# callmeray/PointMVSNet

Measured on AMD Instinct MI355X. Metric: depth-maps/sec (DTU 640x512, 3 src views, 2 flow iters), higher is better.
Workload: dtype f32

## Files before the change

pointmvsnet_amd/csrc/conv3d.hip:

```cpp
#include <stdlib.h>

#include "pf_common.h"
#include "pf_bn_resolve.h"

namespace {

typedef float f32x4 __attribute__((ext_vector_type(4)));

struct ConvGeom {
  int Cin, Cout, Di, Hi, Wi, Do, Ho, Wo;
  int ID, IH, IW, IWP, plane;
  int tiles_d, tiles_h, tiles_w;
  int aff_mode, sps, aff_off;
  const float* in_scale;
  const float* in_shift;
  pf_bn_job in_bn;
};

template <int STRIDE, int TD>
struct Stage {
  static constexpr int ID = (TD - 1) * STRIDE + 3;
  static constexpr int IH = 3 * STRIDE + 3;
  static constexpr int IW = 15 * STRIDE + 3;
  static constexpr int IWP = IW + 1;
  static constexpr int RAW = ID * IH * IWP;
  static constexpr int WANT = STRIDE == 1 ? 16 : 17;
  static constexpr int PLANE = RAW + ((WANT - RAW % 32) + 32) % 32;
  static constexpr int ELEMS = ID * IH * IW;
  static constexpr int NXR = (ELEMS + 63) / 64;
};

template <int NT, int STRIDE, int TD, int MINW>
__global__ __launch_bounds__(256, MINW) void conv3d_k3_kernel(const float* __restrict__ x, const float* __restrict__ wp,
                                                        float* __restrict__ y, ConvGeom g,
                                                        double* __restrict__ partials) {
  using St = Stage<STRIDE, TD>;
  constexpr int ID = St::ID, IH = St::IH, IW = St::IW, IWP = St::IWP, PLANE = St::PLANE;
  constexpr int ELEMS = St::ELEMS, NXR = St::NXR;
  constexpr int NCP = NT * 16;
  constexpr int WSZ = 27 * 4 * NCP;
  constexpr int NWR = (WSZ + 255) / 256;
  constexpr int XS = 4 * PLANE;
  extern __shared__ __attribute__((aligned(16))) float lds[];
  float* xs0 = lds;
  float* ws0 = lds + 2 * XS;
  float* tile = lds;
  double* red = reinterpret_cast<double*>(tile + 4 * NCP * 17 + ((4 * NCP * 17) & 1));

  const int tid = threadIdx.x;
  const int wave = __builtin_amdgcn_readfirstlane(tid >> 6), lane = tid & 63;
  const int li = lane & 15, lk = lane >> 4;
  unsigned xb_, xn_;
  pf_xcd_xy<PF_XCD_CONV3D>(xb_, xn_);
  const int n = (int)xn_, bx = (int)xb_;
  const int plane_i = g.Hi * g.Wi, vol_i = plane_i * g.Di;
  const int64_t plane_o = (int64_t)g.Ho * g.Wo, vol_o = plane_o * g.Do;
  const float* xb = x + (int64_t)n * g.Cin * vol_i;
  float* yb = y + (int64_t)n * g.Cout * vol_o;
  const int cgroups = g.Cin >> 2;

  double ssum[NT], ssq[NT];
#pragma unroll
  for (int t = 0; t < NT; ++t) ssum[t] = ssq[t] = 0.0;

  float* aff = lds + g.aff_off;
  if (g.aff_mode == 1) {
    const int stat = n / g.sps;
    for (int e = tid; e < 2 * g.Cin; e += 256)
      aff[e] = e < g.Cin ? g.in_scale[(int64_t)stat * g.Cin + e] : g.in_shift[(int64_t)stat * g.Cin + e - g.Cin];
  } else if (g.aff_mode == 2) {
    pf_bn_resolve<256>(g.in_bn, n / g.sps, aff, aff + g.Cin, reinterpret_cast<double*>(lds));
  }

  const int total = g.tiles_d * g.tiles_h * g.tiles_w;
  for (int item = bx; item < total; item += gridDim.x) {
    const int tw = item % g.tiles_w;
    const int rest = item / g.tiles_w;
    const int th = rest % g.tiles_h;
    const int td = rest / g.tiles_h;
    const int od0 = td * TD, oh0 = th * 4, ow0 = tw * 16;
    const int id0 = od0 * STRIDE - 1, ih0 = oh0 * STRIDE - 1, iw0 = ow0 * STRIDE - 1;

    unsigned gofs[NXR];
    unsigned okmask = 0;
#pragma unroll
    for (int r = 0; r < NXR; ++r) {
      const int e = lane + 64 * r;
      const int row = e / IW, col = e - row * IW;
      const int dz = row / IH, hy = row - dz * IH;
      const int id = id0 + dz, ih = ih0 + hy, iw = iw0 + col;
      const bool ok = e < ELEMS && id >= 0 && id < g.Di && ih >= 0 && ih < g.Hi && iw >= 0 && iw < g.Wi;
      gofs[r] = ok ? (unsigned)(id * plane_i + ih * g.Wi + iw) : 0u;
      okmask |= (ok ? 1u : 0u) << r;
    }

    float rx[NXR], rw[NWR];
    auto load_group = [&](int cg) {
      const float* src = xb + (int64_t)(cg * 4 + wave) * vol_i;
#pragma unroll
      for (int r = 0; r < NXR; ++r) rx[r] = src[gofs[r]];
      const float* wsrc = wp + (int64_t)cg * WSZ;
#pragma unroll
      for (int r = 0; r < NWR; ++r) {
        const int e = tid + 256 * r;
        rw[r] = (256 * (r + 1) <= WSZ || e < WSZ) ? wsrc[e] : 0.0f;
      }
    };
    auto store_group = [&](int buf, int cg) {
      float* xs = xs0 + buf * XS + wave * PLANE;
      float* ws = ws0 + buf * WSZ;
      float sa = 1.0f, sb = 0.0f;
      if (g.aff_mode) {
        sa = aff[cg * 4 + wave];
        sb = aff[g.Cin + cg * 4 + wave];
      }
#pragma unroll
      for (int r = 0; r < NXR; ++r) {
        const int e = lane + 64 * r;
        float v = rx[r];
        if (g.aff_mode) v = fmaxf(fmaf(v, sa, sb), 0.0f);
        if (64 * (r + 1) <= ELEMS || e < ELEMS) xs[e + e / IW] = ((okmask >> r) & 1u) ? v : 0.0f;
      }
#pragma unroll
      for (int r = 0; r < NWR; ++r) {
        const int e = tid + 256 * r;
        if (256 * (r + 1) <= WSZ || e < WSZ) ws[e] = rw[r];
      }
    };

    f32x4 acc[TD][NT];
#pragma unroll
    for (int d = 0; d < TD; ++d)
#pragma unroll
      for (int t = 0; t < NT; ++t) acc[d][t] = (f32x4){0.0f, 0.0f, 0.0f, 0.0f};

    __syncthreads();
    load_group(0);
    store_group(0, 0);
    __syncthreads();
    for (int cg = 0; cg < cgroups; ++cg) {
      const int buf = cg & 1;
      if (cg + 1 < cgroups) load_group(cg + 1);
      const float* xs = xs0 + buf * XS + lk * PLANE + (wave * STRIDE) * IWP + li * STRIDE;
      const float* ws = ws0 + buf * WSZ + lk * NCP + li;
#pragma unroll
      for (int kd = 0; kd < 3; ++kd) {
#pragma unroll
        for (int kh = 0; kh < 3; ++kh) {
#pragma unroll
          for (int kw = 0; kw < 3; ++kw) {
            const int tap = (kd * 3 + kh) * 3 + kw;
            float b[NT];
#pragma unroll
            for (int t = 0; t < NT; ++t) b[t] = ws[tap * 4 * NCP + 16 * t];
#pragma unroll
            for (int d = 0; d < TD; ++d) {
              const float a = xs[((d * STRIDE + kd) * IH + kh) * IWP + kw];
#pragma unroll
              for (int t = 0; t < NT; ++t) acc[d][t] = __builtin_amdgcn_mfma_f32_16x16x4f32(a, b[t], acc[d][t], 0, 0, 0);
            }
          }
        }
      }
      if (cg + 1 < cgroups) store_group(buf ^ 1, cg + 1);
      __syncthreads();
    }

    const int oh = oh0 + wave;
    float* tl = tile + wave * NCP * 17;
#pragma unroll
    for (int d = 0; d < TD; ++d) {
      const int od = od0 + d;
      const bool row_ok = oh < g.Ho && od < g.Do;
#pragma unroll
      for (int t = 0; t < NT; ++t) {
        float s = 0.0f, q = 0.0f;
#pragma unroll
        for (int r = 0; r < 4; ++r) {
          const int pos = lk * 4 + r;
          const float v = acc[d][t][r];
          tl[(16 * t + li) * 17 + pos] = v;
          if (row_ok && ow0 + pos < g.Wo) {
            s += v;
            q += v * v;
          }
        }
        s += __shfl_xor(s, 16);
        q += __shfl_xor(q, 16);
        s += __shfl_xor(s, 32);
        q += __shfl_xor(q, 32);
        ssum[t] += (double)s;
        ssq[t] += (double)q;
      }
      __builtin_amdgcn_wave_barrier();
      if (row_ok) {
        for (int e = lane; e < NCP * 16; e += 64) {
          const int co = e >> 4, pos = e & 15;
          if (co < g.Cout && ow0 + pos < g.Wo)
            yb[(int64_t)co * vol_o + (int64_t)od * plane_o + (int64_t)oh * g.Wo + ow0 + pos] = tl[co * 17 + pos];
        }
      }
      __builtin_amdgcn_wave_barrier();
    }
  }

  if (partials != nullptr) {
#pragma unroll
    for (int t = 0; t < NT; ++t) {
      if (lane < 16) {
        red[((wave * NCP) + 16 * t + lane) * 2 + 0] = ssum[t];
        red[((wave * NCP) + 16 * t + lane) * 2 + 1] = ssq[t];
      }
    }
    __syncthreads();
    if (tid < g.Cout) {
      double s = 0.0, q = 0.0;
#pragma unroll
      for (int w = 0; w < 4; ++w) {
        s += red[((w * NCP) + tid) * 2 + 0];
        q += red[((w * NCP) + tid) * 2 + 1];
      }
      double* o = partials + (((int64_t)n * gridDim.x + bx) * g.Cout + tid) * 2;
      o[0] = s;
      o[1] = q;
    }
  }
}

template <int COUT>
__global__ __launch_bounds__(256) void conv3d_k3_few_kernel(const float* __restrict__ x, const float* __restrict__ w,
                                                            float* __restrict__ y, int Cin, int D, int H, int W) {
  extern __shared__ __attribute__((aligned(16))) float wl[];
  for (int e = threadIdx.x; e < COUT * Cin * 27; e += 256) wl[e] = w[e];
  __syncthreads();
  const int64_t plane = (int64_t)H * W, vol = plane * D;
  const int64_t i = (int64_t)blockIdx.x * 256 + threadIdx.x;
  const int n = blockIdx.y;
  if (i >= vol) return;
  const int od = (int)(i / plane);
  const int rem = (int)(i - (int64_t)od * plane);
  const int oh = rem / W, ow = rem - oh * W;
  float acc[COUT];
#pragma unroll
  for (int c = 0; c < COUT; ++c) acc[c] = 0.0f;
  const float* xb = x + (int64_t)n * Cin * vol;
  for (int ci = 0; ci < Cin; ++ci) {
    const float* xc = xb + (int64_t)ci * vol;
#pragma unroll
    for (int kd = 0; kd < 3; ++kd) {
      const int id = od + kd - 1;
      const bool dok = id >= 0 && id < D;
#pragma unroll
      for (int kh = 0; kh < 3; ++kh) {
        const int ih = oh + kh - 1;
        const bool hok = dok && ih >= 0 && ih < H;
        const float* row = xc + (int64_t)id * plane + (int64_t)ih * W;
#pragma unroll
        for (int kw = 0; kw < 3; ++kw) {
          const int iw = ow + kw - 1;
          const float v = (hok && iw >= 0 && iw < W) ? row[iw] : 0.0f;
#pragma unroll
          for (int c = 0; c < COUT; ++c) acc[c] = fmaf(v, wl[(c * Cin + ci) * 27 + (kd * 3 + kh) * 3 + kw], acc[c]);
        }
      }
    }
  }
#pragma unroll
  for (int c = 0; c < COUT; ++c) y[((int64_t)n * COUT + c) * vol + i] = acc[c];
}

ConvGeom make_geom(int64_t Cin, int64_t Cout, int64_t Di, int64_t Hi, int64_t Wi, int stride, int td) {
  ConvGeom g;
  g.Cin = (int)Cin;
  g.Cout = (int)Cout;
  g.Di = (int)Di;
  g.Hi = (int)Hi;
  g.Wi = (int)Wi;
  g.Do = (int)((Di - 1) / stride + 1);
  g.Ho = (int)((Hi - 1) / stride + 1);
  g.Wo = (int)((Wi - 1) / stride + 1);
  g.ID = (td - 1) * stride + 3;
  g.IH = 3 * stride + 3;
  g.IW = 15 * stride + 3;
  g.IWP = g.IW + 1;
  const int raw = g.ID * g.IH * g.IWP;
  const int want = stride == 1 ? 16 : 17;
  g.plane = raw + ((want - raw % 32) + 32) % 32;
  g.tiles_d = (g.Do + td - 1) / td;
  g.tiles_h = (g.Ho + 3) / 4;
  g.tiles_w = (g.Wo + 15) / 16;
  g.aff_mode = 0;
  g.sps = 1;
  g.aff_off = 0;
  g.in_scale = g.in_shift = nullptr;
  g.in_bn = pf_bn_job{};
  return g;
}

constexpr size_t kMaxLds = 80 * 1024;

size_t lds_work_bytes(const ConvGeom& g, int NT) {
  const int NCP = NT * 16;
  const size_t staging = sizeof(float) * (size_t)(2 * 4 * g.plane + 2 * 27 * 4 * NCP);
  const size_t epilogue = sizeof(float) * (size_t)(4 * NCP * 17 + 1) + sizeof(double) * (size_t)(4 * NCP * 2);
  const size_t m = staging > epilogue ? staging : epilogue;
  return (m + 15) / 16 * 16;
}
size_t lds_bytes_for(const ConvGeom& g, int NT) {
  return lds_work_bytes(g, NT) + sizeof(float) * 2 * (size_t)g.Cin;
}

int pick_td(int64_t Cin, int64_t Cout, int64_t Di, int64_t Hi, int64_t Wi, int stride) {
  const int NT = (int)((Cout + 15) / 16);
  int best = 0;
  for (int td = (stride == 1 && NT > 1) ? 4 : 2; td >= 1; td >>= 1) {
    const ConvGeom g = make_geom(Cin, Cout, Di, Hi, Wi, stride, td);
    if (lds_bytes_for(g, NT) > kMaxLds) continue;
    best = td;
    if ((int64_t)g.tiles_d * g.tiles_h * g.tiles_w >= 512) return td;
  }
  return best;
}

int blocks_for(const ConvGeom& g) {
  const int64_t total = (int64_t)g.tiles_d * g.tiles_h * g.tiles_w;
#ifndef PF_CONV3D_CAP
#define PF_CONV3D_CAP 2048
#endif
  if (total <= PF_CONV3D_CAP) return (int)total;
  const int64_t per = (total + PF_CONV3D_CAP - 1) / PF_CONV3D_CAP;
  return (int)((total + per - 1) / per);
}

template <int NT, int STRIDE, int TD, int MINW>
int launch(const float* x, const float* wp, float* y, const ConvGeom& g, int64_t N, double* partials,
           hipStream_t s) {
  const size_t lds_bytes = lds_bytes_for(g, NT);
  if (lds_bytes > kMaxLds) return PF_ERR_UNSUPPORTED;
  ConvGeom gk = g;
  gk.aff_off = (int)(lds_work_bytes(g, NT) / sizeof(float));
  if (lds_bytes > 64 * 1024) {
    static std::atomic<unsigned long long> done{0};
    const int rc = pf_allow_big_lds(reinterpret_cast<const void*>(&conv3d_k3_kernel<NT, STRIDE, TD, MINW>),
                                    (int)kMaxLds, done);
    if (rc != PF_OK) return rc;
  }
  dim3 grid((unsigned)blocks_for(g), (unsigned)N);
  hipLaunchKernelGGL((conv3d_k3_kernel<NT, STRIDE, TD, MINW>), grid, dim3(256), lds_bytes, s, x, wp, y, gk, partials);
  return pf_launch_status();
}

template <int NT, int STRIDE, int TD>
int launch_w(const float* x, const float* wp, float* y, const ConvGeom& g, int64_t N, double* partials,
             hipStream_t s) {
  constexpr int kDefault = (NT == 1 && STRIDE == 1 && TD == 2) ? 4 : 2;
  return launch<NT, STRIDE, TD, kDefault>(x, wp, y, g, N, partials, s);
}

template <int NT, int STRIDE>
int launch_td(int td, const float* x, const float* wp, float* y, const ConvGeom& g, int64_t N, double* partials,
              hipStream_t s) {
  if constexpr (STRIDE == 1) {
    if (td == 4) return launch_w<NT, STRIDE, 4>(x, wp, y, g, N, partials, s);
  }
  if (td == 2) return launch_w<NT, STRIDE, 2>(x, wp, y, g, N, partials, s);
  return launch_w<NT, STRIDE, 1>(x, wp, y, g, N, partials, s);
}

}

extern "C" {

int pf_conv3d_blocks(int64_t Cin, int64_t Cout, int64_t Di, int64_t Hi, int64_t Wi, int stride) {
  if (Cin <= 0 || Cout <= 0 || Di <= 0 || Hi <= 0 || Wi <= 0 || (stride != 1 && stride != 2)) return 0;
  const int td = pick_td(Cin, Cout, Di, Hi, Wi, stride);
  if (td == 0) return 0;
  return blocks_for(make_geom(Cin, Cout, Di, Hi, Wi, stride, td));
}

int pf_conv3d_k3_f32(const float* x, const float* wp, float* y, int64_t N, int64_t Cin, int64_t Cout, int64_t Di,
                     int64_t Hi, int64_t Wi, int stride, const float* in_scale, const float* in_shift,
                     const pf_bn_job* in_bn, int samples_per_stat, double* partials, void* stream) {
  PF_REQUIRE(N >= 0 && Cin >= 4 && Cout >= 1 && Di >= 1 && Hi >= 1 && Wi >= 1 && N <= 65535);
  PF_REQUIRE(stride == 1 || stride == 2);
  PF_REQUIRE(samples_per_stat >= 1 && (in_scale == nullptr) == (in_shift == nullptr));
  PF_REQUIRE(in_bn == nullptr || in_scale == nullptr);
  if (in_bn != nullptr && N > 0) {
    PF_REQUIRE(N % samples_per_stat == 0);
    const int rc = pf_bn_in_check(in_bn, (int)Cin, (int)(N / samples_per_stat));
    if (rc != PF_OK) return rc;
  }
  if ((Cin % 4) != 0 || Cout > 32) return PF_ERR_UNSUPPORTED;
  PF_REQUIRE(Cin * Di * Hi * Wi <= INT32_MAX);
  if (N == 0) return PF_OK;
  PF_REQUIRE(x && wp && y);
  const int td = pick_td(Cin, Cout, Di, Hi, Wi, stride);
  if (td == 0) return PF_ERR_UNSUPPORTED;
  ConvGeom g = make_geom(Cin, Cout, Di, Hi, Wi, stride, td);
  g.aff_mode = in_bn ? 2 : (in_scale ? 1 : 0);
  g.sps = samples_per_stat;
  g.in_scale = in_scale;
  g.in_shift = in_shift;
  if (in_bn) g.in_bn = *in_bn;
  hipStream_t s = (hipStream_t)stream;
  const int NT = (int)((Cout + 15) / 16);
  if (stride == 1)
    return NT == 1 ? launch_td<1, 1>(td, x, wp, y, g, N, partials, s) : launch_td<2, 1>(td, x, wp, y, g, N, partials, s);
  return NT == 1 ? launch_td<1, 2>(td, x, wp, y, g, N, partials, s) : launch_td<2, 2>(td, x, wp, y, g, N, partials, s);
}

int pf_conv3d_k3_few_f32(const float* x, const float* w, float* y, int64_t N, int64_t Cin, int64_t Cout, int64_t D,
                         int64_t H, int64_t W, void* stream) {
  PF_REQUIRE(N >= 0 && Cin >= 1 && Cout >= 1 && D >= 1 && H >= 1 && W >= 1 && N <= 65535);
  if (Cout > 4 || Cout * Cin * 27 * sizeof(float) > 48 * 1024) return PF_ERR_UNSUPPORTED;
  PF_REQUIRE(H * W <= INT32_MAX);
  if (N == 0) return PF_OK;
  PF_REQUIRE(x && w && y);
  const size_t lds = sizeof(float) * (size_t)(Cout * Cin * 27);
  dim3 grid((unsigned)pf_cdiv(D * H * W, 256), (unsigned)N);
  hipStream_t s = (hipStream_t)stream;
  switch ((int)Cout) {
    case 1: hipLaunchKernelGGL(conv3d_k3_few_kernel<1>, grid, dim3(256), lds, s, x, w, y, (int)Cin, (int)D, (int)H, (int)W); break;
    case 2: hipLaunchKernelGGL(conv3d_k3_few_kernel<2>, grid, dim3(256), lds, s, x, w, y, (int)Cin, (int)D, (int)H, (int)W); break;
    case 3: hipLaunchKernelGGL(conv3d_k3_few_kernel<3>, grid, dim3(256), lds, s, x, w, y, (int)Cin, (int)D, (int)H, (int)W); break;
    default: hipLaunchKernelGGL(conv3d_k3_few_kernel<4>, grid, dim3(256), lds, s, x, w, y, (int)Cin, (int)D, (int)H, (int)W); break;
  }
  return pf_launch_status();
}

}
```

pointmvsnet_amd/csrc/conv3d_pair.hip:

```cpp
#include <stdlib.h>

#include "pf_common.h"

namespace {

typedef float f32x4 __attribute__((ext_vector_type(4)));

struct PairGeom {
  int Cin, Cout, D, H, W;
  int tiles_d, tiles_h, tiles_w;
};

template <int TD>
struct PStage {
  static constexpr int ID = TD + 2;
  static constexpr int IH = 10;
  static constexpr int IW = 18;
  static constexpr int IWP = IW + 1;
  static constexpr int RAW = ID * IH * IWP;
  static constexpr int PLANE = RAW + ((16 - RAW % 32) + 32) % 32;
  static constexpr int ELEMS = ID * IH * IW;
  static constexpr int NXR = (ELEMS + 63) / 64;
};

constexpr int kTaps = 36;
constexpr int kWsz = kTaps * 4 * 16;

template <int TD>
constexpr size_t pair_lds_bytes() {
  using St = PStage<TD>;
  const size_t staging = sizeof(float) * (size_t)(2 * 4 * St::PLANE + 2 * kWsz);
  const size_t epilogue = sizeof(float) * (size_t)(4 * 16 * 17 + 1) + sizeof(double) * (size_t)(4 * 16 * 2);
  return staging > epilogue ? staging : epilogue;
}

template <int TD, int MINW>
__global__ __launch_bounds__(256, MINW) void conv3d_k3_pair_kernel(const float* __restrict__ x,
                                                                   const float* __restrict__ wp,
                                                                   float* __restrict__ y, PairGeom g,
                                                                   double* __restrict__ partials) {
  using St = PStage<TD>;
  constexpr int ID = St::ID, IH = St::IH, IW = St::IW, IWP = St::IWP, PLANE = St::PLANE;
  constexpr int ELEMS = St::ELEMS, NXR = St::NXR;
  constexpr int NWR = (kWsz + 255) / 256;
  constexpr int XS = 4 * PLANE;
  extern __shared__ __attribute__((aligned(16))) float lds[];
  float* xs0 = lds;
  float* ws0 = lds + 2 * XS;
  float* tile = lds;
  double* red = reinterpret_cast<double*>(tile + 4 * 16 * 17 + ((4 * 16 * 17) & 1));

  const int tid = threadIdx.x;
  const int wave = __builtin_amdgcn_readfirstlane(tid >> 6), lane = tid & 63;
  const int li = lane & 15, lk = lane >> 4;
  unsigned xb_, xn_;
  pf_xcd_xy<PF_XCD_CONV3D>(xb_, xn_);
  const int n = (int)xn_, bx = (int)xb_;
  const int plane_i = g.H * g.W, vol = plane_i * g.D;
  const float* xb = x + (int64_t)n * g.Cin * vol;
  float* yb = y + (int64_t)n * g.Cout * vol;
  const int cgroups = g.Cin >> 2;

  double ssum = 0.0, ssq = 0.0;

  const int total = g.tiles_d * g.tiles_h * g.tiles_w;
  for (int item = bx; item < total; item += gridDim.x) {
    const int tw = item % g.tiles_w;
    const int rest = item / g.tiles_w;
    const int th = rest % g.tiles_h;
    const int td = rest / g.tiles_h;
    const int od0 = td * TD, oh0 = th * 8, ow0 = tw * 16;
    const int id0 = od0 - 1, ih0 = oh0 - 1, iw0 = ow0 - 1;

    unsigned gofs[NXR];
    unsigned okmask = 0;
#pragma unroll
    for (int r = 0; r < NXR; ++r) {
      const int e = lane + 64 * r;
      const int row = e / IW, col = e - row * IW;
      const int dz = row / IH, hy = row - dz * IH;
      const int id = id0 + dz, ih = ih0 + hy, iw = iw0 + col;
      const bool ok = e < ELEMS && id >= 0 && id < g.D && ih >= 0 && ih < g.H && iw >= 0 && iw < g.W;
      gofs[r] = ok ? (unsigned)(id * plane_i + ih * g.W + iw) : 0u;
      okmask |= (ok ? 1u : 0u) << r;
    }

    float rx[NXR], rw[NWR];
    auto load_group = [&](int cg) {
      const float* src = xb + (int64_t)(cg * 4 + wave) * vol;
#pragma unroll
      for (int r = 0; r < NXR; ++r) rx[r] = src[gofs[r]];
      const float* wsrc = wp + (int64_t)cg * kWsz;
#pragma unroll
      for (int r = 0; r < NWR; ++r) {
        const int e = tid + 256 * r;
        rw[r] = (256 * (r + 1) <= kWsz || e < kWsz) ? wsrc[e] : 0.0f;
      }
    };
    auto store_group = [&](int buf) {
      float* xs = xs0 + buf * XS + wave * PLANE;
      float* ws = ws0 + buf * kWsz;
#pragma unroll
      for (int r = 0; r < NXR; ++r) {
        const int e = lane + 64 * r;
        if (64 * (r + 1) <= ELEMS || e < ELEMS) xs[e + e / IW] = ((okmask >> r) & 1u) ? rx[r] : 0.0f;
      }
#pragma unroll
      for (int r = 0; r < NWR; ++r) {
        const int e = tid + 256 * r;
        if (256 * (r + 1) <= kWsz || e < kWsz) ws[e] = rw[r];
      }
    };

    f32x4 acc[TD];
#pragma unroll
    for (int d = 0; d < TD; ++d) acc[d] = (f32x4){0.0f, 0.0f, 0.0f, 0.0f};

    __syncthreads();
    load_group(0);
    store_group(0);
    __syncthreads();
    for (int cg = 0; cg < cgroups; ++cg) {
      const int buf = cg & 1;
      if (cg + 1 < cgroups) load_group(cg + 1);
      const float* xs = xs0 + buf * XS + lk * PLANE + (2 * wave) * IWP + li;
      const float* ws = ws0 + buf * kWsz + lk * 16 + li;
#pragma unroll
      for (int kd = 0; kd < 3; ++kd) {
#pragma unroll
        for (int kh = 0; kh < 4; ++kh) {
#pragma unroll
          for (int kw = 0; kw < 3; ++kw) {
            const int tap = (kd * 4 + kh) * 3 + kw;
            const float b = ws[tap * 4 * 16];
#pragma unroll
            for (int d = 0; d < TD; ++d) {
              const float a = xs[((d + kd) * IH + kh) * IWP + kw];
              acc[d] = __builtin_amdgcn_mfma_f32_16x16x4f32(a, b, acc[d], 0, 0, 0);
            }
          }
        }
      }
      if (cg + 1 < cgroups) store_group(buf ^ 1);
      __syncthreads();
    }

    const int oh = oh0 + 2 * wave + (li >> 3);
    float* tl = tile + wave * 16 * 17;
#pragma unroll
    for (int d = 0; d < TD; ++d) {
      const int od = od0 + d;
      const bool row_ok = oh < g.H && od < g.D;
      float s = 0.0f, q = 0.0f;
#pragma unroll
      for (int r = 0; r < 4; ++r) {
        const int pos = lk * 4 + r;
        const float v = acc[d][r];
        tl[li * 17 + pos] = v;
        if (row_ok && ow0 + pos < g.W) {
          s += v;
          q += v * v;
        }
      }
      s += __shfl_xor(s, 8);
      q += __shfl_xor(q, 8);
      s += __shfl_xor(s, 16);
      q += __shfl_xor(q, 16);
      s += __shfl_xor(s, 32);
      q += __shfl_xor(q, 32);
      ssum += (double)s;
      ssq += (double)q;
      __builtin_amdgcn_wave_barrier();
      if (od < g.D) {
        for (int e = lane; e < 16 * 16; e += 64) {
          const int col = e >> 4, pos = e & 15;
          const int co = col & 7, ohh = oh0 + 2 * wave + (col >> 3);
          if (co < g.Cout && ohh < g.H && ow0 + pos < g.W)
            yb[(int64_t)co * vol + (int64_t)od * plane_i + (int64_t)ohh * g.W + ow0 + pos] = tl[col * 17 + pos];
        }
      }
      __builtin_amdgcn_wave_barrier();
    }
  }

  if (partials != nullptr) {
    if (lane < 8) {
      red[(wave * 16 + lane) * 2 + 0] = ssum;
      red[(wave * 16 + lane) * 2 + 1] = ssq;
    }
    __syncthreads();
    if (tid < g.Cout) {
      double s = 0.0, q = 0.0;
#pragma unroll
      for (int w = 0; w < 4; ++w) {
        s += red[(w * 16 + tid) * 2 + 0];
        q += red[(w * 16 + tid) * 2 + 1];
      }
      double* o = partials + (((int64_t)n * gridDim.x + bx) * g.Cout + tid) * 2;
      o[0] = s;
      o[1] = q;
    }
  }
}

#ifndef PF_PAIR_TD
#define PF_PAIR_TD 2
#endif
#ifndef PF_PAIR_MINW
#define PF_PAIR_MINW 3
#endif
constexpr int kPairTD = PF_PAIR_TD;

PairGeom make_pair_geom(int64_t Cin, int64_t Cout, int64_t D, int64_t H, int64_t W) {
  PairGeom g;
  g.Cin = (int)Cin;
  g.Cout = (int)Cout;
  g.D = (int)D;
  g.H = (int)H;
  g.W = (int)W;
  g.tiles_d = (g.D + kPairTD - 1) / kPairTD;
  g.tiles_h = (g.H + 7) / 8;
  g.tiles_w = (g.W + 15) / 16;
  return g;
}

int pair_blocks(const PairGeom& g) {
  const int64_t total = (int64_t)g.tiles_d * g.tiles_h * g.tiles_w;
#ifndef PF_CONV3D_CAP
#define PF_CONV3D_CAP 2048
#endif
  if (total <= PF_CONV3D_CAP) return (int)total;
  const int64_t per = (total + PF_CONV3D_CAP - 1) / PF_CONV3D_CAP;
  return (int)((total + per - 1) / per);
}

}

extern "C" {

int pf_conv3d_pair_blocks(int64_t Cin, int64_t Cout, int64_t D, int64_t H, int64_t W) {
  if (Cin <= 0 || Cout <= 0 || Cout > 8 || D <= 0 || H <= 0 || W <= 0) return 0;
  return pair_blocks(make_pair_geom(Cin, Cout, D, H, W));
}

int pf_conv3d_k3_pair_f32(const float* x, const float* wp, float* y, int64_t N, int64_t Cin, int64_t Cout, int64_t D,
                          int64_t H, int64_t W, double* partials, void* stream) {
  PF_REQUIRE(N >= 0 && Cin >= 4 && Cout >= 1 && D >= 1 && H >= 1 && W >= 1 && N <= 65535);
  if ((Cin % 4) != 0 || Cout > 8) return PF_ERR_UNSUPPORTED;
  PF_REQUIRE(Cin * D * H * W <= INT32_MAX);
  if (N == 0) return PF_OK;
  PF_REQUIRE(x && wp && y);
  const PairGeom g = make_pair_geom(Cin, Cout, D, H, W);
  constexpr size_t lds_bytes = pair_lds_bytes<kPairTD>();
  static_assert(lds_bytes <= 64 * 1024, "pair tile must fit the default dynamic LDS limit");
  dim3 grid((unsigned)pair_blocks(g), (unsigned)N);
  hipLaunchKernelGGL((conv3d_k3_pair_kernel<kPairTD, PF_PAIR_MINW>), grid, dim3(256), lds_bytes, (hipStream_t)stream, x, wp, y, g,
                     partials);
  return pf_launch_status();
}

}
```

pointmvsnet_amd/csrc/pf_common.h:

```cpp
#pragma once

#include <hip/hip_runtime.h>
#include <stdint.h>

#include "pointflow_hip.h"

#define PF_WAVE 64

unsigned* pf_status_ptr();

#define PF_REQUIRE(cond)                 \
  do {                                   \
    if (!(cond)) return PF_ERR_INVALID_ARG; \
  } while (0)

#define PF_HIP(expr)                        \
  do {                                      \
    hipError_t _e = (expr);                 \
    if (_e != hipSuccess) return (int)_e;   \
  } while (0)

static inline int pf_launch_status() {
  hipError_t e = hipGetLastError();
  return e == hipSuccess ? PF_OK : (int)e;
}

static inline int64_t pf_cdiv(int64_t a, int64_t b) { return (a + b - 1) / b; }

#include <atomic>
static inline int pf_allow_big_lds(const void* kernel, int bytes, std::atomic<unsigned long long>& flags) {
  int dev = 0;
  PF_HIP(hipGetDevice(&dev));
  const unsigned long long bit = 1ull << (dev & 63);
  if (flags.load(std::memory_order_acquire) & bit) return PF_OK;
  PF_HIP(hipFuncSetAttribute(kernel, hipFuncAttributeMaxDynamicSharedMemorySize, bytes));
  flags.fetch_or(bit, std::memory_order_release);
  return PF_OK;
}

#if defined(__HIPCC__)
static __global__ __launch_bounds__(256) void pf_zero_kernel(unsigned* __restrict__ p, size_t words) {
  const size_t stride = (size_t)gridDim.x * 256;
  for (size_t i = (size_t)blockIdx.x * 256 + threadIdx.x; i < words; i += stride) p[i] = 0u;
}
static inline int pf_zero_async(void* p, size_t bytes, hipStream_t s) {
  if (bytes == 0) return PF_OK;
  const size_t words = bytes / 4;
  size_t blocks = (words + 255) / 256;
  if (blocks > 4096) blocks = 4096;
  hipLaunchKernelGGL(pf_zero_kernel, dim3((unsigned)blocks), dim3(256), 0, s, reinterpret_cast<unsigned*>(p), words);
  const hipError_t e = hipGetLastError();
  return e == hipSuccess ? PF_OK : (int)e;
}
#endif

#ifndef PF_XCD
#define PF_XCD 1
#endif
#define PF_XCD_TOWER 1
#define PF_XCD_CONV3D 2
#define PF_XCD_FETCH 4
#define PF_XCD_KNN 8
#define PF_XCD_EDGE 16
#define PF_XCD_FRUSTUM 32
#ifdef __HIPCC__
__device__ __forceinline__ unsigned pf_xcd_chunk(unsigned lin, unsigned total) {
  const unsigned per = total >> 3, rem = total & 7u;
  const unsigned x = lin & 7u, j = lin >> 3;
  return x * per + (x < rem ? x : rem) + j;
}
__device__ __forceinline__ unsigned pf_xcd_band(unsigned b, unsigned tiles_per_plane) {
  if ((tiles_per_plane & 7u) != 0u) return b;
  const unsigned band = tiles_per_plane >> 3;
  const unsigned x = b & 7u, j = b >> 3;
  const unsigned d = j / band, o = j - d * band;
  return d * tiles_per_plane + x * band + o;
}
template <int FAMILY>
__device__ __forceinline__ void pf_xcd_xy(unsigned& bx, unsigned& by) {
  if ((PF_XCD & FAMILY) == 0) {
    bx = blockIdx.x;
    by = blockIdx.y;
    return;
  }
  const unsigned gx = gridDim.x;
  const unsigned L = pf_xcd_chunk(blockIdx.y * gx + blockIdx.x, gx * gridDim.y);
  by = L / gx;
  bx = L - by * gx;
}
#endif

struct PfTaps {
  int off[4];
  float wgt[4];
  bool ok[4];
  int xi, yi;
  float fx, fy;
};

__device__ __forceinline__ void pf_project_taps(float X, float Y, float Z, const float* __restrict__ Kv,
                                                const float* __restrict__ Ev, int H, int W, PfTaps& t) {
  float px = X, py = Y, pz = Z;
  if (Ev != nullptr) {
    px = fmaf(Ev[2], Z, fmaf(Ev[1], Y, Ev[0] * X)) + Ev[3];
    py = fmaf(Ev[6], Z, fmaf(Ev[5], Y, Ev[4] * X)) + Ev[7];
    pz = fmaf(Ev[10], Z, fmaf(Ev[9], Y, Ev[8] * X)) + Ev[11];
  }
  const float nx = px / pz;
  const float ny = py / pz;
  const float u = fmaf(Kv[2], 1.0f, fmaf(Kv[1], ny, Kv[0] * nx));
  const float v = fmaf(Kv[5], 1.0f, fmaf(Kv[4], ny, Kv[3] * nx));
  const float gx = ((u - 0.5f) / (float)(W - 1)) * 2.0f - 1.0f;
  const float gy = ((v - 0.5f) / (float)(H - 1)) * 2.0f - 1.0f;
  const float ix = (gx + 1.0f) * ((float)(W - 1) / 2.0f);
  const float iy = (gy + 1.0f) * ((float)(H - 1) / 2.0f);
  const float x0 = floorf(ix), y0 = floorf(iy);
  const float wx1 = ix - x0, wy1 = iy - y0;
  const float wx0 = 1.0f - wx1, wy0 = 1.0f - wy1;
  const float xmax = (float)(W - 1), ymax = (float)(H - 1);
  const bool vx0 = (x0 >= 0.0f) && (x0 <= xmax);
  const bool vx1 = (x0 + 1.0f >= 0.0f) && (x0 + 1.0f <= xmax);
  const bool vy0 = (y0 >= 0.0f) && (y0 <= ymax);
  const bool vy1 = (y0 + 1.0f >= 0.0f) && (y0 + 1.0f <= ymax);
  const int xi = (vx0 || vx1) ? (int)x0 : 0;
  const int yi = (vy0 || vy1) ? (int)y0 : 0;
  t.xi = xi;
  t.yi = yi;
  t.fx = wx1;
  t.fy = wy1;
  t.ok[0] = vy0 && vx0;
  t.ok[1] = vy0 && vx1;
  t.ok[2] = vy1 && vx0;
  t.ok[3] = vy1 && vx1;
  t.off[0] = t.ok[0] ? yi * W + xi : 0;
  t.off[1] = t.ok[1] ? yi * W + xi + 1 : 0;
  t.off[2] = t.ok[2] ? (yi + 1) * W + xi : 0;
  t.off[3] = t.ok[3] ? (yi + 1) * W + xi + 1 : 0;
  t.wgt[0] = t.ok[0] ? wy0 * wx0 : 0.0f;
  t.wgt[1] = t.ok[1] ? wy0 * wx1 : 0.0f;
  t.wgt[2] = t.ok[2] ? wy1 * wx0 : 0.0f;
  t.wgt[3] = t.ok[3] ? wy1 * wx1 : 0.0f;
}

__device__ __forceinline__ float pf_sample(const float* __restrict__ plane, const PfTaps& t) {
  const float a = plane[t.off[0]];
  const float b = plane[t.off[1]];
  const float c = plane[t.off[2]];
  const float d = plane[t.off[3]];
  return ((a * t.wgt[0] + b * t.wgt[1]) + c * t.wgt[2]) + d * t.wgt[3];
}

__device__ __forceinline__ float pf_flow_confidence(const float* __restrict__ prob, int i, int hw) {
  float p[5];
#pragma unroll
  for (int d = 0; d < 5; ++d) p[d] = prob[(int64_t)d * hw + i];
  const double a0 = (double)p[0] * -2.0, a1 = (double)p[1] * -1.0, a2 = (double)p[2] * 0.0;
  const double a3 = (double)p[3] * 1.0, a4 = (double)p[4] * 2.0;
  const double idx = (a0 + (((a1 + a2) + a3) + a4)) + 2.0;
  int fl = (int)floor(idx);
  int ce = fl + 1;
  ce = ce < 0 ? 0 : (ce > 4 ? 4 : ce);
  fl = fl < 0 ? fl + 5 : fl;
  fl = fl < 0 ? 0 : (fl > 4 ? 4 : fl);
  return p[fl] + p[ce];
}
```

Measured before the change: 1090.

## Software-pipeline LDS fetches with MFMA and band conv3d tiles per XCD

Restructures the inner tap loops of the stride-2 single-tile conv3d and the pair conv3d kernels so that LDS operands for the next tap group are double-buffered in registers while the current group's MFMAs run, with sched_barriers fixing the order. It also turns on XCD-aware tile remapping for conv3d (PF_XCD=3) using a new depth/height banding function, so neighbouring tiles that share halos land on the same XCD for L2 reuse. Global loads now use byte offsets with a scalarised channel base to save address arithmetic. The extra register buffers raise VGPR pressure and could lower occupancy.

```diff
diff --git a/pointmvsnet_amd/csrc/conv3d.hip b/pointmvsnet_amd/csrc/conv3d.hip
--- a/pointmvsnet_amd/csrc/conv3d.hip
+++ b/pointmvsnet_amd/csrc/conv3d.hip
@@ -50,9 +50,7 @@
   const int tid = threadIdx.x;
   const int wave = __builtin_amdgcn_readfirstlane(tid >> 6), lane = tid & 63;
   const int li = lane & 15, lk = lane >> 4;
-  unsigned xb_, xn_;
-  pf_xcd_xy<PF_XCD_CONV3D>(xb_, xn_);
-  const int n = (int)xn_, bx = (int)xb_;
+  const int n = blockIdx.y, bx = (int)pf_xcd_dband(blockIdx.x, gridDim.x, (unsigned)g.tiles_h, (unsigned)g.tiles_w);
   const int plane_i = g.Hi * g.Wi, vol_i = plane_i * g.Di;
   const int64_t plane_o = (int64_t)g.Ho * g.Wo, vol_o = plane_o * g.Do;
   const float* xb = x + (int64_t)n * g.Cin * vol_i;
@@ -90,15 +88,16 @@
       const int dz = row / IH, hy = row - dz * IH;
       const int id = id0 + dz, ih = ih0 + hy, iw = iw0 + col;
       const bool ok = e < ELEMS && id >= 0 && id < g.Di && ih >= 0 && ih < g.Hi && iw >= 0 && iw < g.Wi;
-      gofs[r] = ok ? (unsigned)(id * plane_i + ih * g.Wi + iw) : 0u;
+      gofs[r] = ok ? 4u * (unsigned)(id * plane_i + ih * g.Wi + iw) : 0u;
       okmask |= (ok ? 1u : 0u) << r;
     }
 
     float rx[NXR], rw[NWR];
     auto load_group = [&](int cg) {
-      const float* src = xb + (int64_t)(cg * 4 + wave) * vol_i;
-#pragma unroll
-      for (int r = 0; r < NXR; ++r) rx[r] = src[gofs[r]];
+      const int ch = __builtin_amdgcn_readfirstlane(cg * 4 + wave);
+      const char* src = reinterpret_cast<const char*>(xb + (int64_t)ch * vol_i);
+#pragma unroll
+      for (int r = 0; r < NXR; ++r) rx[r] = *reinterpret_cast<const float*>(src + gofs[r]);
       const float* wsrc = wp + (int64_t)cg * WSZ;
 #pragma unroll
       for (int r = 0; r < NWR; ++r) {
@@ -140,9 +139,34 @@
     __syncthreads();
     for (int cg = 0; cg < cgroups; ++cg) {
       const int buf = cg & 1;
-      if (cg + 1 < cgroups) load_group(cg + 1);
       const float* xs = xs0 + buf * XS + lk * PLANE + (wave * STRIDE) * IWP + li * STRIDE;
       const float* ws = ws0 + buf * WSZ + lk * NCP + li;
+      if constexpr (STRIDE == 2 && NT == 1) {
+        float a[2][TD][3], b[2][3];
+        auto fetch = [&](int st) {
+#pragma unroll
+          for (int kw = 0; kw < 3; ++kw) {
+            b[st & 1][kw] = ws[(st * 3 + kw) * 4 * NCP];
+#pragma unroll
+            for (int d = 0; d < TD; ++d) a[st & 1][d][kw] = xs[((d * STRIDE + st / 3) * IH + st % 3) * IWP + kw];
+          }
+        };
+        fetch(0);
+        if (cg + 1 < cgroups) load_group(cg + 1);
+#pragma unroll
+        for (int st = 0; st < 9; ++st) {
+          if (st < 8) fetch(st + 1);
+          __builtin_amdgcn_sched_barrier(0);
+#pragma unroll
+          for (int kw = 0; kw < 3; ++kw) {
+#pragma unroll
+            for (int d = 0; d < TD; ++d)
+              acc[d][0] = __builtin_amdgcn_mfma_f32_16x16x4f32(a[st & 1][d][kw], b[st & 1][kw], acc[d][0], 0, 0, 0);
+          }
+          __builtin_amdgcn_sched_barrier(0);
+        }
+      } else {
+      if (cg + 1 < cgroups) load_group(cg + 1);
 #pragma unroll
       for (int kd = 0; kd < 3; ++kd) {
 #pragma unroll
@@ -161,6 +185,7 @@
             }
           }
         }
+      }
       }
       if (cg + 1 < cgroups) store_group(buf ^ 1, cg + 1);
       __syncthreads();
diff --git a/pointmvsnet_amd/csrc/conv3d_pair.hip b/pointmvsnet_amd/csrc/conv3d_pair.hip
--- a/pointmvsnet_amd/csrc/conv3d_pair.hip
+++ b/pointmvsnet_amd/csrc/conv3d_pair.hip
@@ -53,9 +53,7 @@
   const int tid = threadIdx.x;
   const int wave = __builtin_amdgcn_readfirstlane(tid >> 6), lane = tid & 63;
   const int li = lane & 15, lk = lane >> 4;
-  unsigned xb_, xn_;
-  pf_xcd_xy<PF_XCD_CONV3D>(xb_, xn_);
-  const int n = (int)xn_, bx = (int)xb_;
+  const int n = blockIdx.y, bx = (int)pf_xcd_dband(blockIdx.x, gridDim.x, (unsigned)g.tiles_h, (unsigned)g.tiles_w);
   const int plane_i = g.H * g.W, vol = plane_i * g.D;
   const float* xb = x + (int64_t)n * g.Cin * vol;
   float* yb = y + (int64_t)n * g.Cout * vol;
@@ -81,15 +79,16 @@
       const int dz = row / IH, hy = row - dz * IH;
       const int id = id0 + dz, ih = ih0 + hy, iw = iw0 + col;
       const bool ok = e < ELEMS && id >= 0 && id < g.D && ih >= 0 && ih < g.H && iw >= 0 && iw < g.W;
-      gofs[r] = ok ? (unsigned)(id * plane_i + ih * g.W + iw) : 0u;
+      gofs[r] = ok ? 4u * (unsigned)(id * plane_i + ih * g.W + iw) : 0u;
       okmask |= (ok ? 1u : 0u) << r;
     }
 
     float rx[NXR], rw[NWR];
     auto load_group = [&](int cg) {
-      const float* src = xb + (int64_t)(cg * 4 + wave) * vol;
-#pragma unroll
-      for (int r = 0; r < NXR; ++r) rx[r] = src[gofs[r]];
+      const int ch = __builtin_amdgcn_readfirstlane(cg * 4 + wave);
+      const char* src = reinterpret_cast<const char*>(xb + (int64_t)ch * vol);
+#pragma unroll
+      for (int r = 0; r < NXR; ++r) rx[r] = *reinterpret_cast<const float*>(src + gofs[r]);
       const float* wsrc = wp + (int64_t)cg * kWsz;
 #pragma unroll
       for (int r = 0; r < NWR; ++r) {
@@ -122,24 +121,31 @@
     __syncthreads();
     for (int cg = 0; cg < cgroups; ++cg) {
       const int buf = cg & 1;
-      if (cg + 1 < cgroups) load_group(cg + 1);
       const float* xs = xs0 + buf * XS + lk * PLANE + (2 * wave) * IWP + li;
       const float* ws = ws0 + buf * kWsz + lk * 16 + li;
-#pragma unroll
-      for (int kd = 0; kd < 3; ++kd) {
-#pragma unroll
-        for (int kh = 0; kh < 4; ++kh) {
-#pragma unroll
-          for (int kw = 0; kw < 3; ++kw) {
-            const int tap = (kd * 4 + kh) * 3 + kw;
-            const float b = ws[tap * 4 * 16];
-#pragma unroll
-            for (int d = 0; d < TD; ++d) {
-              const float a = xs[((d + kd) * IH + kh) * IWP + kw];
-              acc[d] = __builtin_amdgcn_mfma_f32_16x16x4f32(a, b, acc[d], 0, 0, 0);
-            }
-          }
-        }
+      float a[2][TD][6], b[2][6];
+      auto fetch = [&](int st) {
+#pragma unroll
+        for (int t = 0; t < 6; ++t) {
+          const int kd = st >> 1, kh = 2 * (st & 1) + t / 3, kw = t % 3;
+          b[st & 1][t] = ws[((kd * 4 + kh) * 3 + kw) * 4 * 16];
+#pragma unroll
+          for (int d = 0; d < TD; ++d) a[st & 1][d][t] = xs[((d + kd) * IH + kh) * IWP + kw];
+        }
+      };
+      fetch(0);
+      if (cg + 1 < cgroups) load_group(cg + 1);
+#pragma unroll
+      for (int st = 0; st < 6; ++st) {
+        if (st < 5) fetch(st + 1);
+        __builtin_amdgcn_sched_barrier(0);
+#pragma unroll
+        for (int t = 0; t < 6; ++t) {
+#pragma unroll
+          for (int d = 0; d < TD; ++d)
+            acc[d] = __builtin_amdgcn_mfma_f32_16x16x4f32(a[st & 1][d][t], b[st & 1][t], acc[d], 0, 0, 0);
+        }
+        __builtin_amdgcn_sched_barrier(0);
       }
       if (cg + 1 < cgroups) store_group(buf ^ 1);
       __syncthreads();
diff --git a/pointmvsnet_amd/csrc/pf_common.h b/pointmvsnet_amd/csrc/pf_common.h
--- a/pointmvsnet_amd/csrc/pf_common.h
+++ b/pointmvsnet_amd/csrc/pf_common.h
@@ -55,7 +55,7 @@
 #endif
 
 #ifndef PF_XCD
-#define PF_XCD 1
+#define PF_XCD 3
 #endif
 #define PF_XCD_TOWER 1
 #define PF_XCD_CONV3D 2
@@ -75,6 +75,15 @@
   const unsigned x = b & 7u, j = b >> 3;
   const unsigned d = j / band, o = j - d * band;
   return d * tiles_per_plane + x * band + o;
+}
+__device__ __forceinline__ unsigned pf_xcd_dband(unsigned b, unsigned G, unsigned tiles_h, unsigned tiles_w) {
+  const unsigned per_d = tiles_h * tiles_w;
+  if ((PF_XCD & PF_XCD_CONV3D) == 0 || (tiles_h & 7u) != 0u || G % per_d != 0u) return b;
+  const unsigned gd = G / per_d, band = tiles_h >> 3;
+  const unsigned x = b & 7u, j = b >> 3;
+  const unsigned td = j % gd, r = j / gd;
+  const unsigned hl = r % band, tw = r / band;
+  return (td * tiles_h + x * band + hl) * tiles_w + tw;
 }
 template <int FAMILY>
 __device__ __forceinline__ void pf_xcd_xy(unsigned& bx, unsigned& by) {
```

New measurement: 1081. Within noise of the previous version (-0.9%).
